# AbrahamSanders/realtime-codec-agent

Hardware: AMD Instinct MI355X
Metric: batch-encode audio-hours/hour (+ xRT and p50 frame-step latency of 1 duplex stream in `duplex`) (higher is better)
Workload: dtype f32; 1 GPU; batch MagiCodec-style encode, 16 kHz stereo, 0.1 s chunks / 2.0 s context, 256 windows per step (BASELINE configs[1]); codebook=131072x16

## Files before the change

realtime_codec_agent_amd/csrc/rca_codec.hip:

```cpp
#include <stdarg.h>

#include <algorithm>
#include <array>
#include <cmath>
#include <map>
#include <type_traits>

#include "rca_common.h"
#include "rca_conv_balance.h"

namespace rca {
thread_local char g_err[512] = {0};
}
using namespace rca;

typedef float f32x16 __attribute__((ext_vector_type(16)));

#define RCA_LAT_MAX_FRAMES 64
#define RCA_LDS_BUDGET (152 * 1024)

typedef float f32x4 __attribute__((ext_vector_type(4)));

struct RowSrc {
    const float* base;
// ... 1864 lines not shown
        float xv[NS][7];
        bool exists[NS];
        int cell[NS];
#pragma unroll
        for (int q = 0; q < NS; ++q) {
            const int tr = tid + 256 * q;
            const int t = t_start + tr;
            exists[q] = tr < WIN && t >= 0 && t < Lin;
            cell[q] = tr < WIN ? (tr % S) * SLOTS + tr / S : -1;
#pragma unroll
            for (int kk = 0; kk < 7; ++kk) {
                const int i = t + kk - 3;
                xv[q][kk] = (tr < WIN && i >= 0 && i < fsrc.T) ? xr[i] : 0.0f;
            }
        }
#pragma unroll
        for (int cb = 0; cb < CPS; ++cb)
#pragma unroll
            for (int h = 0; h < 2; ++h) {
                unsigned hi[NS][4], lo[NS][4];
#pragma unroll
                for (int j = 0; j < 4; ++j) {
                    float v[NS][2];
#pragma unroll
                    for (int e = 0; e < 2; ++e) {
                        const float* wr = w_in8 + (cb * 16 + 8 * h + 2 * j + e) * 8;
                        const float w0 = wr[0], w1 = wr[1], w2 = wr[2], w3 = wr[3], w4 = wr[4], w5 = wr[5], w6 = wr[6], bi = wr[7];
#pragma unroll
                        for (int q = 0; q < NS; ++q) {
                            float a = bi;
#if RCA_BLK_ABL == 1
                            v[q][e] = xv[q][e]; continue;
#endif
                            a = __builtin_fmaf(w0, xv[q][0], a); a = __builtin_fmaf(w1, xv[q][1], a); a = __builtin_fmaf(w2, xv[q][2], a);
                            a = __builtin_fmaf(w3, xv[q][3], a); a = __builtin_fmaf(w4, xv[q][4], a); a = __builtin_fmaf(w5, xv[q][5], a);
                            a = __builtin_fmaf(w6, xv[q][6], a);
                            a = in_act ? fmaxf(a, a * slope) : a;
                            v[q][e] = exists[q] ? a : 0.0f;
                        }
                    }
#pragma unroll
                    for (int q = 0; q < NS; ++q) {
                        hi[q][j] = conv_pack_bf16x2(v[q][0], v[q][1]);
                        if (SPLIT) lo[q][j] = conv_pack_bf16x2(v[q][0] - __uint_as_float(hi[q][j] << 16), v[q][1] - __uint_as_float(hi[q][j] & 0xffff0000u));
                    }
                }
#pragma unroll
                for (int q = 0; q < NS; ++q)
                    if (cell[q] >= 0) {
                        blk_lds[(cb * NPL) * CELLS + h * S * SLOTS + cell[q]] = conv_u32x4{hi[q][0], hi[q][1], hi[q][2], hi[q][3]};
                        if (SPLIT) blk_lds[(cb * NPL + 1) * CELLS + h * S * SLOTS + cell[q]] = conv_u32x4{lo[q][0], lo[q][1], lo[q][2], lo[q][3]};
                    }
            }
    } else {
        stage_load(0);
        stage_write(0);
    }
    __syncthreads();
    int f = 0;
    for (int st = 0; st < nstages; ++st) {
        const int buf = SB ? 0 : (st & 1);
        constexpr int LOAD_AT = CPS * KS - PD;
#pragma unroll
        for (int cb = 0; cb < CPS; ++cb) {
            const conv_u32x4* xb = blk_lds + ((buf * CPS + cb) * NPL) * CELLS;
#pragma unroll
            for (int kk = 0; kk < KS; ++kk) {
                if (cb * KS + kk == LOAD_AT && st + 1 < nstages) stage_load(st + 1);
                const int slot = (cb * KS + kk) % PD;
                const int cell = bcell0 + (kk % S) * SLOTS + kk / S;
                conv_u32x4 bh[4], bl[4];
#pragma unroll
                for (int wn = 0; wn < 4; ++wn) {
                    bh[wn] = xb[cell + wn * 32];
                    if (SPLIT) bl[wn] = xb[CELLS + cell + wn * 32];
                }
                conv_u32x4 a_h[WMT], a_l[WMT];
#pragma unroll
                for (int wm = 0; wm < WMT; ++wm) { a_h[wm] = ah[slot][wm]; if (SPLIT) a_l[wm] = al[slot][wm]; }
                {
                    const long fn = (long)min(f + PD, nfrag - 1) * 64;
#pragma unroll
                    for (int wm = 0; wm < WMT; ++wm) {
                        ah[slot][wm] = wq_hi[wm * wtile + fn];
                        if (SPLIT) al[slot][wm] = wq_lo[wm * wtile + fn];
                    }
                }
                ++f;
#if RCA_BLK_ABL == 2
                asm volatile("" ::"v"(a_h[0]), "v"(bh[0]), "v"(bh[1]), "v"(bh[2]), "v"(bh[3]));
                continue;
#endif
#pragma unroll
                for (int wm = 0; wm < WMT; ++wm)
#pragma unroll
                    for (int wn = 0; wn < 4; ++wn)
                        acc[wm][wn] = __builtin_amdgcn_mfma_f32_32x32x16_bf16(__builtin_bit_cast(conv_bf16x8, a_h[wm]), __builtin_bit_cast(conv_bf16x8, bh[wn]), acc[wm][wn], 0, 0, 0);
                if (SPLIT) {
#pragma unroll
                    for (int wm = 0; wm < WMT; ++wm)
#pragma unroll
                        for (int wn = 0; wn < 4; ++wn)
                            acc[wm][wn] = __builtin_amdgcn_mfma_f32_32x32x16_bf16(__builtin_bit_cast(conv_bf16x8, a_h[wm]), __builtin_bit_cast(conv_bf16x8, bl[wn]), acc[wm][wn], 0, 0, 0);
#pragma unroll
                    for (int wm = 0; wm < WMT; ++wm)
#pragma unroll
                        for (int wn = 0; wn < 4; ++wn)
                            acc[wm][wn] = __builtin_amdgcn_mfma_f32_32x32x16_bf16(__builtin_bit_cast(conv_bf16x8, a_l[wm]), __builtin_bit_cast(conv_bf16x8, bh[wn]), acc[wm][wn], 0, 0, 0);
                }
            }
        }
        if (SB) __syncthreads();
        if (st + 1 < nstages) stage_write(SB ? 0 : (buf ^ 1));
        __syncthreads();
    }
#if RCA_BLK_ABL == 3
    if (lane == 0 && acc[0][0][0] + acc[0][1][1] + acc[WMT - 1][2][2] + acc[WMT - 1][3][3] == 12345.0f) y_hi[0] = 1;
    return;
#endif
#pragma unroll
    for (int wn = 0; wn < 4; ++wn)
#pragma unroll
    for (int wm = 0; wm < WMT; ++wm) {
        const int t = n0 + wn_w * 128 + wn * 32 + n;
        if (t >= Lout) continue;
        if (OUT == 1) {
            float* yr = y_f32 + ((long)b * Cout + co0 + wm * 32 + 4 * half) * Lout + t;
#pragma unroll
            for (int r = 0; r < 16; ++r) yr[(long)((r & 3) + 8 * (r >> 2)) * Lout] = acc[wm][wn][r];
        } else {
            const int Cbo = Cout / 16;
#pragma unroll
            for (int g = 0; g < 4; ++g) {
                float v[4];
#pragma unroll
                for (int j = 0; j < 4; ++j) {
                    const float a = acc[wm][wn][4 * g + j];
                    v[j] = act ? fmaxf(a, a * slope) : a;
                }
                const int ch = co0 + wm * 32 + 8 * g + 4 * half;
                const long o = (((long)b * Cbo + ch / 16) * Lout + t) * 16 + (ch & 15);
                const unsigned h0 = conv_pack_bf16x2(v[0], v[1]), h1 = conv_pack_bf16x2(v[2], v[3]);
                *reinterpret_cast<uint2*>(y_hi + o) = make_uint2(h0, h1);
                if (SPLIT) {
                    const unsigned l0 = conv_pack_bf16x2(v[0] - __uint_as_float(h0 << 16), v[1] - __uint_as_float(h0 & 0xffff0000u));
                    const unsigned l1 = conv_pack_bf16x2(v[2] - __uint_as_float(h1 << 16), v[3] - __uint_as_float(h1 & 0xffff0000u));
                    *reinterpret_cast<uint2*>(y_lo + o) = make_uint2(l0, l1);
                }
            }
        }
    }
}

struct Bf16Pack { conv_bf16raw* hi = nullptr; conv_bf16raw* lo = nullptr; float* w_in8 = nullptr; };

struct rca_codec {
    rca_codec_config_t cfg;
    int device = 0;
    hipStream_t stream = nullptr;
    int hop = 1;
    int variant = 1;
    int mfma_mode = 0;
    bool lat_mode = false;
    int enc_left_frames = 0, dec_left_frames = 0;
    bool window_trim = false;
    std::vector<ConvLayer> enc, dec;
    std::vector<Bf16Pack> bf16_packs;
    bool bf16_blk_split = true;
    float *q_in_w = nullptr, *q_in_b = nullptr;
    float *cb = nullptr, *hc = nullptr, *cbp = nullptr;
    DevBuf act[2], zbuf, keys, io_a, io_b, tail;
    void* pin = nullptr; size_t pin_cap = 0;
    struct StreamGraph { hipGraphExec_t exec = nullptr; int seen = 0; unsigned long long sig = 0; };
    std::map<std::array<int, 5>, StreamGraph> sgraphs;
    bool stream_graphs = true;
    std::map<std::array<long, 4>, float*> ingest_tabs;
    int* err_flag = nullptr;
    hipStream_t last_stream = nullptr;
    bool last_stream_valid = false;
    hipEvent_t xev = nullptr;
    struct Prof { hipEvent_t a, b; int kclass; double flops, bytes; };
    bool profile = false;
    std::vector<Prof> prof;
    std::vector<Prof> prof_pool;
};

struct ProfScope {
    rca_codec* h; hipStream_t st; rca_codec::Prof p; bool on;
    ProfScope(rca_codec* h_, hipStream_t st_, int kclass, double flops, double bytes) : h(h_), st(st_), on(h_->profile) {
        if (!on) return;
        if (!h->prof_pool.empty()) { p = h->prof_pool.back(); h->prof_pool.pop_back(); }
        else { (void)hipEventCreate(&p.a); (void)hipEventCreate(&p.b); }
        p.kclass = kclass; p.flops = flops; p.bytes = bytes;
        (void)hipEventRecord(p.a, st);
    }
    ~ProfScope() {
        if (!on) return;
        (void)hipEventRecord(p.b, st);
        h->prof.push_back(p);
    }
};

static int upload(const rca_tensor_t* ts, int n, const std::string& name, long numel, float** out) {
    const rca_tensor_t* t = find_tensor(ts, n, name);
    if (!t) return fail(RCA_ERR_MISSING, "tensor '%s' missing", name.c_str());
    if (t->numel != numel) return fail(RCA_ERR_ARG, "tensor '%s': numel %ld, expected %ld", name.c_str(), (long)t->numel, numel);
    if (t->dtype != RCA_F32) return fail(RCA_ERR_ARG, "tensor '%s' must be f32", name.c_str());
    RCA_HIP(hipMalloc((void**)out, (size_t)numel * sizeof(float)));
    RCA_HIP(hipMemcpy(*out, t->data, (size_t)numel * sizeof(float), hipMemcpyHostToDevice));
    return RCA_OK;
}

static int pack_weights_cic(const float* w_host, const ConvLayer& L, int cic, float** out, int* nchunks_out) {
    const int K = L.cin * L.k;
    const int nchunks = (L.cin + cic - 1) / cic;
    const int Kpad = nchunks * cic * L.k;
    const int cout_pad = (L.cout + 127) / 128 * 128;
    const long n = (long)(cout_pad / 32) * (Kpad / 8) * 64 * 4;
    std::vector<float> p((size_t)n, 0.0f);
    for (int cot = 0; cot < cout_pad / 32; ++cot)
        for (int q = 0; q < Kpad / 8; ++q)
            for (int lane = 0; lane < 64; ++lane)
                for (int e = 0; e < 4; ++e) {
                    const int co = cot * 32 + (lane & 31);
                    const int k = 2 * (4 * q + e) + (lane >> 5);
                    float v = 0.0f;
                    if (co < L.cout && k < K) v = w_host[(long)co * K + k];
                    p[(((long)cot * (Kpad / 8) + q) * 64 + lane) * 4 + e] = v;
                }
    RCA_HIP(hipMalloc((void**)out, (size_t)n * sizeof(float)));
    RCA_HIP(hipMemcpy(*out, p.data(), (size_t)n * sizeof(float), hipMemcpyHostToDevice));
    *nchunks_out = nchunks;
    return RCA_OK;
}
static int pack_weights(const float* w_host, ConvLayer& L) {
    L.K = L.cin * L.k;
    L.cout_pad = (L.cout + 127) / 128 * 128;
    int rc = pack_weights_cic(w_host, L, conv_cic(L.k, L.s), &L.wp, &L.nchunks);
    if (rc != RCA_OK) return rc;
    L.Kpad = L.nchunks * conv_cic(L.k, L.s) * L.k;
    return pack_weights_cic(w_host, L, conv_cic_ws(L.k, L.s), &L.wp2, &L.nchunks2);
}

static int pack_weights_tr(const float* w_host, ConvLayer& L) {
    const int cic = 16, K = 2 * L.cin;
    const int nchunks = (L.cin + cic - 1) / cic;
    const int Kpad = nchunks * cic * 2;
    L.cout_pad = (L.cout + 127) / 128 * 128;
    const long per_phase = (long)(L.cout_pad / 32) * (Kpad / 8) * 64 * 4;
    std::vector<float> p((size_t)per_phase * L.s, 0.0f);
    for (int r = 0; r < L.s; ++r)
        for (int cot = 0; cot < L.cout_pad / 32; ++cot)
            for (int q = 0; q < Kpad / 8; ++q)
                for (int lane = 0; lane < 64; ++lane)
                    for (int e = 0; e < 4; ++e) {
                        const int co = cot * 32 + (lane & 31);
                        const int k = 2 * (4 * q + e) + (lane >> 5);
                        float v = 0.0f;
                        if (co < L.cout && k < K) {
                            const int ci = k >> 1, j = k & 1;
                            v = w_host[((long)ci * L.cout + co) * L.k + r + j * L.s];
                        }
                        p[r * per_phase + (((long)cot * (Kpad / 8) + q) * 64 + lane) * 4 + e] = v;
                    }
    RCA_HIP(hipMalloc((void**)&L.wp_tr, p.size() * sizeof(float)));
    RCA_HIP(hipMemcpy(L.wp_tr, p.data(), p.size() * sizeof(float), hipMemcpyHostToDevice));
    {
        std::vector<float> t((size_t)L.cin * L.cout * L.k);
        for (int ci = 0; ci < L.cin; ++ci)
            for (int co = 0; co < L.cout; ++co)
                for (int kk = 0; kk < L.k; ++kk) t[((size_t)co * L.k + kk) * L.cin + ci] = w_host[((size_t)ci * L.cout + co) * L.k + kk];
        RCA_HIP(hipMalloc((void**)&L.w_lat, t.size() * sizeof(float)));
        RCA_HIP(hipMemcpy(L.w_lat, t.data(), t.size() * sizeof(float), hipMemcpyHostToDevice));
    }
    L.nchunks_tr = nchunks;
    return RCA_OK;
}

static bool mfma_supported(int k, int s) {
    return (k == 4 && s == 2) || (k == 8 && s == 4) || (k == 10 && s == 5) || (k == 16 && s == 8) || (k == 3 && s == 1);
}

extern "C" const char* rca_last_error(void) { return g_err; }
extern "C" const char* rca_version(void) { return "rca-hip 0.1 (gfx950)"; }
extern "C" int rca_device_sync(int32_t device) {
    RCA_HIP(hipSetDevice(device));
    RCA_HIP(hipDeviceSynchronize());
    return RCA_OK;
}

extern "C" int rca_device_count(int* n) {
    if (!n) return fail(RCA_ERR_ARG, "null");
    RCA_HIP(hipGetDeviceCount(n));
    return RCA_OK;
}

extern "C" int rca_codec_destroy(rca_codec_t* h) {
#ifdef RCA_CONV_TIMELINE
    if (h && getenv("RCA_CONV_TIMELINE_OUT")) {
        long* b = nullptr;
        unsigned n = 6 << 16;
        (void)hipDeviceSynchronize();
        (void)hipMemcpyFromSymbol(&b, HIP_SYMBOL(rca_prof_buf), 8);
        if (b) {
            std::vector<long> host((size_t)(6 << 16) * 8);
            (void)hipMemcpy(host.data(), b, host.size() * 8, hipMemcpyDeviceToHost);
// ... 416 lines not shown
    const double cflops = 2.0 * L.cin * L.k * L.cout * (double)B * Lout;
    const double cbytes = 4.0 * ((double)B * L.cin * Lin + (double)B * L.cout * Lout + (double)L.cin * L.k * L.cout);
    if (view > 0 && view < Lout) {
        const int Lv = view;
        const double vin = std::min((double)Lin, (double)Lv * L.s + L.k - L.s);
        ProfScope ps(h, st, 0, 2.0 * L.cin * L.k * L.cout * (double)B * Lv,
                     4.0 * ((double)B * L.cin * vin + (double)B * L.cout * Lv + (double)L.cin * L.k * L.cout));
        const float* xv = x + (long)(Lout - Lv) * L.s;
        const int act = ((L.pre && !in_activated) ? 1 : 0) | (want_post ? 2 : 0);
        if (post_done) *post_done = want_post;
        if (L.k == 4 && L.s == 2) return launch_conv_mfma<4, 2, 4>(L, xv, y, B, Lin, Lv, slope, st, nullptr, act, 0);
        if (L.k == 8 && L.s == 4) return launch_conv_mfma<8, 4, RCA_CIC_K8>(L, xv, y, B, Lin, Lv, slope, st, nullptr, act, 0);
        if (L.k == 10 && L.s == 5) return launch_conv_mfma<10, 5, 4>(L, xv, y, B, Lin, Lv, slope, st, nullptr, act, 0);
        if (L.k == 16 && L.s == 8) return launch_conv_mfma<16, 8, RCA_CIC_K16>(L, xv, y, B, Lin, Lv, slope, st, nullptr, act, 0);
        if ((long)cdiv((long)B * Lv, 32) * cdiv(L.cout, 32) <= 1024 && L.cin % 16 == 0) {
            launch_conv_cfg<3, 1, 16, 1, 1, 0, 0>(L, L.wp, L.cin / 16, xv, y, Lin, Lv, (long)B * Lv, slope, FuseIn{}, TrInfo{}, st, act);
            RCA_LAUNCH_CHECK();
            return RCA_OK;
        }
        return launch_conv_mfma<3, 1, RCA_CIC_K3>(L, xv, y, B, Lin, Lv, slope, st, nullptr, act, 0);
    }
    if (mfma_conv_ok(h, L, B, Lin, clamp_out)) {
        ProfScope ps(h, st, 0, cflops, cbytes);
        if (h->variant == 2 && try_conv_ws(L, x, y, B, Lin, Lout, slope, st, nullptr)) { RCA_LAUNCH_CHECK(); return RCA_OK; }
        const int act = ((L.pre && !in_activated) ? 1 : 0) | (want_post ? 2 : 0);
        if (post_done) *post_done = want_post;
        if (L.k == 4 && L.s == 2) return launch_conv_mfma<4, 2, 4>(L, x, y, B, Lin, Lout, slope, st, nullptr, act, h->mfma_mode);
        if (L.k == 8 && L.s == 4) return launch_conv_mfma<8, 4, RCA_CIC_K8>(L, x, y, B, Lin, Lout, slope, st, nullptr, act, h->mfma_mode);
        if (L.k == 10 && L.s == 5) return launch_conv_mfma<10, 5, 4>(L, x, y, B, Lin, Lout, slope, st, nullptr, act, h->mfma_mode);
        if (L.k == 16 && L.s == 8) return launch_conv_mfma<16, 8, RCA_CIC_K16>(L, x, y, B, Lin, Lout, slope, st, nullptr, act, h->mfma_mode);
        if (L.k == 3 && L.s == 1) return launch_conv_mfma<3, 1, RCA_CIC_K3>(L, x, y, B, Lin, Lout, slope, st, nullptr, act, h->mfma_mode);
    }
    if (in_activated) return fail(RCA_ERR_ARG, "internal: activated input handed to a kernel without that mode");
    const long total = (long)B * L.cout * Lout;
    ProfScope ps(h, st, 3, cflops, cbytes);
    conv1d_chain_kernel<<<cdiv(total, 256), 256, 0, st>>>(x, L.w, L.b, y, B, L.cin, Lin, L.cout, Lout, L.k, L.s, L.pre, slope, clamp_out);
    RCA_LAUNCH_CHECK();
    return RCA_OK;
}

static int pack_weights_bf16(const ConvLayer& L, Bf16Pack* out) {
    const long nw = (long)L.cout * L.cin * L.k;
    std::vector<float> w(nw);
    RCA_HIP(hipMemcpy(w.data(), L.w, nw * 4, hipMemcpyDeviceToHost));
    const int ncot = L.cout / 32, ncb = L.cin / 16;
    std::vector<conv_bf16raw> hi((size_t)ncot * ncb * L.k * 64 * 8), lo(hi.size());
    auto rne = [](float f) { unsigned u; memcpy(&u, &f, 4); u += 0x7FFFu + ((u >> 16) & 1u); return (conv_bf16raw)(u >> 16); };
    auto up = [](conv_bf16raw h) { unsigned u = (unsigned)h << 16; float f; memcpy(&f, &u, 4); return f; };
    for (int cot = 0; cot < ncot; ++cot)
        for (int cb = 0; cb < ncb; ++cb)
            for (int kk = 0; kk < L.k; ++kk)
                for (int lane = 0; lane < 64; ++lane)
                    for (int j = 0; j < 8; ++j) {
                        const int co = cot * 32 + (lane & 31), ci = cb * 16 + 8 * (lane >> 5) + j;
                        const float v = w[((long)co * L.cin + ci) * L.k + kk];
                        const size_t o = ((((size_t)cot * ncb + cb) * L.k + kk) * 64 + lane) * 8 + j;
                        hi[o] = rne(v);
                        lo[o] = rne(v - up(hi[o]));
                    }
    RCA_HIP(hipMalloc((void**)&out->hi, hi.size() * 2));
    RCA_HIP(hipMalloc((void**)&out->lo, lo.size() * 2));
    RCA_HIP(hipMemcpy(out->hi, hi.data(), hi.size() * 2, hipMemcpyHostToDevice));
    RCA_HIP(hipMemcpy(out->lo, lo.data(), lo.size() * 2, hipMemcpyHostToDevice));
    return RCA_OK;
}

template <int KS, int S, int WGM, int CPS, int OUT, int FUSE = 0, int WMT = 1>
static int launch_conv_bf16(bool split, const ConvLayer& L, const Bf16Pack& wp, const conv_bf16raw* xh, const conv_bf16raw* xl, conv_bf16raw* yh,
                            conv_bf16raw* yl, float* yf, int B, int Lin, int act, float slope, hipStream_t st, RowSrc fsrc = RowSrc{},
                            const float* w_in8 = nullptr, int in_act = 0) {
    constexpr int WGN = 4 / WGM, NT = 128 * WGN;
    constexpr int SLOTS = NT + (KS - 1) / S;
    const int Lout = Lin / S;
    const int n_ct = cdiv(Lout, NT), n_cot = L.cout / (32 * WGM * (split ? 1 : WMT));
    const dim3 grid((unsigned)(((long)n_ct * B + 7) / 8 * 8 * n_cot));
    const int nstages = L.cin / 16 / CPS;
    const size_t lds = (size_t)((nstages > 1 && !(split && S >= 5)) ? 2 : 1) * CPS * (split ? 2 : 1) * 2 * S * SLOTS * 16;
    if (split) {
        auto k = conv_bf16_blk_kernel<KS, S, WGM, CPS, 1, OUT, FUSE, 1>;
        static bool attr = false;
        if (!attr) { (void)hipFuncSetAttribute((const void*)k, hipFuncAttributeMaxDynamicSharedMemorySize, (int)lds); attr = true; }
        k<<<grid, 256, lds, st>>>(xh, xl, wp.hi, wp.lo, L.b, yh, yl, yf, L.cin, Lin, L.cout, Lout, act, slope, B, n_ct, n_cot, fsrc, w_in8, in_act);
    } else {
        auto k = conv_bf16_blk_kernel<KS, S, WGM, CPS, 0, OUT, FUSE, WMT>;
        static bool attr = false;
        if (!attr) { (void)hipFuncSetAttribute((const void*)k, hipFuncAttributeMaxDynamicSharedMemorySize, (int)lds); attr = true; }
        k<<<grid, 256, lds, st>>>(xh, xl, wp.hi, wp.lo, L.b, yh, yl, yf, L.cin, Lin, L.cout, Lout, act, slope, B, n_ct, n_cot, fsrc, w_in8, in_act);
    }
    RCA_LAUNCH_CHECK();
    return RCA_OK;
}

static bool bf16_blk_layer_ok(const ConvLayer& L, bool last) {
    if (L.tr || L.cin % 16 || L.cout % 64) return false;
    if (last) return L.k == 3 && L.s == 1 && L.cin % 64 == 0 && L.cout % 128 == 0;
    if (L.k == 4 && L.s == 2) return L.cin % 32 == 0;
    if ((L.k == 8 && L.s == 4) || (L.k == 10 && L.s == 5) || (L.k == 16 && L.s == 8)) return L.cout % 128 == 0;
    return false;
}
static bool bf16_blk_ok(const rca_codec* h, int tap_layer) {
    const size_t n = h->enc.size();
    if (h->mfma_mode == 0 || h->lat_mode || h->variant != 1 || n < 3) return false;
    if (h->mfma_mode == 3 && !h->bf16_blk_split) return false;
    if (tap_layer >= 0 && tap_layer != (int)n - 1) return false;
    if (h->enc[0].k != 7 || h->enc[0].cin != 1 || h->enc[0].cout % 16 || h->enc[0].cout > 64) return false;
    for (size_t li = 1; li < n; ++li)
        if (!bf16_blk_layer_ok(h->enc[li], li + 1 == n)) return false;
    return true;
}
static int run_encoder_bf16(rca_codec* h, RowSrc src, int B, int Tp, size_t max_elems, hipStream_t st, float** ze_out, int tap_layer, float* tap_dev,
                            int bf16_tap = -1, const conv_bf16raw** bf16_planes = nullptr) {
    const bool split = h->mfma_mode == 3;
    const float slope = h->cfg.leaky_slope;
    const size_t n = h->enc.size();
    int rc;
    if (h->bf16_packs.size() != n) {
        h->bf16_packs.assign(n, Bf16Pack{});
        for (size_t li = 1; li < n; ++li)
            if ((rc = pack_weights_bf16(h->enc[li], &h->bf16_packs[li])) != RCA_OK) return rc;
        const ConvLayer& L0 = h->enc[0];
        std::vector<float> w0((size_t)L0.cout * L0.k), b0(L0.cout), t8((size_t)L0.cout * 8, 0.0f);
        RCA_HIP(hipMemcpy(w0.data(), L0.w, w0.size() * 4, hipMemcpyDeviceToHost));
        RCA_HIP(hipMemcpy(b0.data(), L0.b, b0.size() * 4, hipMemcpyDeviceToHost));
        for (int co = 0; co < L0.cout; ++co) {
            for (int kk = 0; kk < L0.k; ++kk) t8[(size_t)co * 8 + kk] = w0[(size_t)co * L0.k + kk];
            t8[(size_t)co * 8 + 7] = b0[co];
        }
        RCA_HIP(hipMalloc((void**)&h->bf16_packs[0].w_in8, t8.size() * 4));
        RCA_HIP(hipMemcpy(h->bf16_packs[0].w_in8, t8.data(), t8.size() * 4, hipMemcpyHostToDevice));
    }
    auto hi_of = [&](int buf) { return h->act[buf].as<conv_bf16raw>(); };
    auto lo_of = [&](int buf) { return h->act[buf].as<conv_bf16raw>() + max_elems; };
    const double esz = split ? 4.0 : 2.0;
    int cur = 0, L = Tp;
    const bool fuse_in = h->enc[1].k == 4 && h->enc[1].s == 2 && h->enc[0].cout == 32 && !getenv("RCA_BF16_NO_FUSE_IN");
    if (bf16_tap >= 0 && (bf16_tap + 1 >= (int)n || (bf16_tap == 0 && fuse_in)))
        return fail(RCA_ERR_ARG, "bf16 tap: layer %d is not materialised (conv_in fused: %d, last layer: %d, f32)", bf16_tap, (int)fuse_in, (int)n - 1);
    auto stop_at = [&](int li) {
        if (li != bf16_tap) return false;
        bf16_planes[0] = hi_of(cur);
        bf16_planes[1] = lo_of(cur);
        return true;
    };
    if (!fuse_in) {
        const ConvLayer& L0 = h->enc[0];
        const long total = (long)B * L;
        ProfScope ps(h, st, 2, 2.0 * L0.k * L0.cout * (double)total, 4.0 * (double)total + esz * (double)total * L0.cout);
        const int act = h->enc[1].pre ? 1 : 0;
        if (split) conv_in_blk_kernel<7, 1><<<dim3(cdiv(L, 256), B), 256, 0, st>>>(src, h->bf16_packs[0].w_in8, L0.b, hi_of(cur), lo_of(cur), B, L0.cout, L, act, slope);
        else conv_in_blk_kernel<7, 0><<<dim3(cdiv(L, 256), B), 256, 0, st>>>(src, h->bf16_packs[0].w_in8, L0.b, hi_of(cur), lo_of(cur), B, L0.cout, L, act, slope);
        RCA_LAUNCH_CHECK();
        if (stop_at(0)) return RCA_OK;
    }
    for (size_t li = 1; li < n; ++li) {
        const ConvLayer& Ly = h->enc[li];
        const bool last = li + 1 == n;
        const int Lout = L / Ly.s;
        const int act = (!last && h->enc[li + 1].pre) ? 1 : 0;
        const bool fused_li = li == 1 && fuse_in;
        ProfScope ps(h, st, 0, 2.0 * Ly.cin * Ly.k * Ly.cout * (double)B * Lout + (fused_li ? 2.0 * h->enc[0].k * h->enc[0].cout * (double)B * L : 0.0),
                     (fused_li ? 4.0 * (double)B * L : esz * (double)B * Ly.cin * L) + (last ? 4.0 : esz) * (double)B * Ly.cout * Lout +
                         esz * (double)Ly.cin * Ly.k * Ly.cout);
        const Bf16Pack& wp = h->bf16_packs[li];
        const conv_bf16raw *xh = hi_of(cur), *xl = lo_of(cur);
        conv_bf16raw *yh = hi_of(cur ^ 1), *yl = lo_of(cur ^ 1);
        float* yf = h->act[cur ^ 1].as<float>();
        if (!split && Ly.k == 10 && Ly.cout % 256 == 0) rc = launch_conv_bf16<10, 5, 4, 1, 0, 0, 2>(split, Ly, wp, xh, xl, yh, yl, yf, B, L, act, slope, st);
        else if (last) rc = launch_conv_bf16<3, 1, 4, 4, 1>(split, Ly, wp, xh, xl, yh, yl, yf, B, L, act, slope, st);
        else if (Ly.k == 4 && li == 1 && fuse_in)
            rc = launch_conv_bf16<4, 2, 2, 2, 0, 1>(split, Ly, wp, xh, xl, yh, yl, yf, B, L, act, slope, st, src, h->bf16_packs[0].w_in8, Ly.pre ? 1 : 0);
        else if (Ly.k == 4) rc = launch_conv_bf16<4, 2, 2, 2, 0>(split, Ly, wp, xh, xl, yh, yl, yf, B, L, act, slope, st);
        else if (Ly.k == 8) rc = launch_conv_bf16<8, 4, 4, 1, 0>(split, Ly, wp, xh, xl, yh, yl, yf, B, L, act, slope, st);
        else if (Ly.k == 10) rc = launch_conv_bf16<10, 5, 4, 1, 0>(split, Ly, wp, xh, xl, yh, yl, yf, B, L, act, slope, st);
        else rc = launch_conv_bf16<16, 8, 4, 1, 0>(split, Ly, wp, xh, xl, yh, yl, yf, B, L, act, slope, st);
        if (rc != RCA_OK) return rc;
        L = Lout;
        cur ^= 1;
        if (last && tap_layer == (int)li) RCA_HIP(hipMemcpyAsync(tap_dev, yf, (size_t)B * Ly.cout * L * 4, hipMemcpyDeviceToDevice, st));
        if (stop_at((int)li)) return RCA_OK;
    }
    *ze_out = h->act[cur].as<float>();
    return RCA_OK;
}

static int run_encoder(rca_codec* h, RowSrc src, int B, hipStream_t st, float** ze_out, int* F_out, int tap_layer, float* tap_dev,
                       int bf16_tap = -1, const conv_bf16raw** bf16_planes = nullptr, int keep = 0, int* Fz_out = nullptr) {
    const rca_codec_config_t& c = h->cfg;
    const int F = (src.T + h->hop - 1) / h->hop;
    const int Tp = F * h->hop;
    if (F < 1) return fail(RCA_ERR_ARG, "empty audio (T=%d)", src.T);
    if (Fz_out) *Fz_out = F;
    size_t max_elems = 0;
    {
        long L = Tp;
        max_elems = std::max(max_elems, (size_t)B * c.channels[0] * L);
        for (int i = 0; i < c.n_stages; ++i) { L /= c.strides[i]; max_elems = std::max(max_elems, (size_t)B * c.channels[i + 1] * L); }
        max_elems = std::max(max_elems, (size_t)B * c.latent_dim * L);
    }
    int rc;
    if ((rc = h->act[0].ensure(max_elems * 4)) != RCA_OK) return rc;
    if ((rc = h->act[1].ensure(max_elems * 4)) != RCA_OK) return rc;
    if (bf16_blk_ok(h, tap_layer) && (double)B * max_elems < 4.0e18 && Tp / h->enc[1].s >= 64) {
        *F_out = F;
        return run_encoder_bf16(h, src, B, Tp, max_elems, st, ze_out, tap_layer, tap_dev, bf16_tap, bf16_planes);
    }
    if (bf16_tap >= 0) return fail(RCA_ERR_ARG, "bf16 tap: encode() does not take the blocked bf16 pipeline here (mfma mode %d, B=%d T=%d)", h->mfma_mode, B, src.T);
    int cur = 0;
    int L = Tp;
    size_t first = 1;
    const ConvLayer& E0 = h->enc[0];
    const ConvLayer& E1 = h->enc[1];
    const bool fuse01 = !h->lat_mode && h->variant >= 1 && tap_layer != 0 && E0.k == 7 && E1.wp && E1.k == 2 * E1.s && (double)B * E1.cin * L < 4.0e9 &&
                        ((E1.k == 4 && E1.s == 2) || (E1.k == 8 && E1.s == 4) || (E1.k == 16 && E1.s == 8)) && L / E1.s >= 67 &&
                        (double)E1.cout * (L / E1.s) < 2.6e8 &&
                        (src.row_off ? (double)src.span : (double)src.C * (double)std::labs(src.chan_stride) + (double)std::labs(src.win_stride) + src.T) < 5.0e8;
    bool prev_post = false;
    auto handoff = [&](size_t next, int Lnext) {
        return tap_layer < 0 && h->variant == 1 && !h->lat_mode && next < h->enc.size() && h->enc[next].pre && mfma_conv_ok(h, h->enc[next], B, Lnext, 0);
    };
    if (fuse01) {
        float* y = h->act[cur].as<float>();
        FuseIn fin{src, E0.w, E0.b};
        const float slope = c.leaky_slope;
        const int Lout = L / E1.s;
        {
            ProfScope ps(h, st, 0, 2.0 * E1.cin * E1.k * E1.cout * (double)B * Lout + 2.0 * E0.k * E0.cout * (double)B * L,
                         4.0 * ((double)B * src.T + (double)B * E1.cout * Lout + (double)E1.cin * E1.k * E1.cout));
            prev_post = handoff(2, Lout);
            const int act = (E1.pre ? 1 : 0) | (prev_post ? 2 : 0);
            if (h->variant == 2 && try_conv_ws(E1, nullptr, y, B, L, Lout, slope, st, &fin)) { rc = RCA_OK; RCA_LAUNCH_CHECK(); }
            else if (E1.k == 4) rc = launch_conv_mfma<4, 2, 4>(E1, nullptr, y, B, L, Lout, slope, st, &fin, act, h->mfma_mode);
            else if (E1.k == 8) rc = launch_conv_mfma<8, 4, RCA_CIC_K8>(E1, nullptr, y, B, L, Lout, slope, st, &fin, act, h->mfma_mode);
            else rc = launch_conv_mfma<16, 8, RCA_CIC_K16>(E1, nullptr, y, B, L, Lout, slope, st, &fin, act, h->mfma_mode);
        }
        if (rc != RCA_OK) return rc;
        L = Lout;
        first = 2;
        if (tap_layer == 1) RCA_HIP(hipMemcpyAsync(tap_dev, y, (size_t)B * E1.cout * L * 4, hipMemcpyDeviceToDevice, st));
    } else if (h->lat_mode && !src.row_off && src.win_stride == 0 && src.C == B &&
               try_conv_lds(h, h->enc[0], src.base, src.chan_stride, src.T, h->act[cur].as<float>(), B, L, 0, st)) {
        RCA_LAUNCH_CHECK();
    } else {
        const ConvLayer& L0 = h->enc[0];
        const long total = (long)B * L;
        float* y = h->act[cur].as<float>();
        ProfScope ps(h, st, 2, 2.0 * L0.k * L0.cout * (double)total, 4.0 * ((double)total + (double)total * L0.cout));
        if (L0.k == 7) conv_in_kernel<7><<<cdiv(total, 256), 256, 0, st>>>(src, L0.w, L0.b, y, B, L0.cout, L);
        else if (L0.k == 5) conv_in_kernel<5><<<cdiv(total, 256), 256, 0, st>>>(src, L0.w, L0.b, y, B, L0.cout, L);
        else conv_in_kernel<3><<<cdiv(total, 256), 256, 0, st>>>(src, L0.w, L0.b, y, B, L0.cout, L);
        RCA_LAUNCH_CHECK();
        if (tap_layer == 0) RCA_HIP(hipMemcpyAsync(tap_dev, y, (size_t)B * L0.cout * L * 4, hipMemcpyDeviceToDevice, st));
    }
    for (size_t li = first; li < h->enc.size(); ++li) {
        const ConvLayer& Ly = h->enc[li];
        float* x = h->act[cur].as<float>();
        float* y = h->act[cur ^ 1].as<float>();
        bool done = false;
        int view = 0;
        if (li + 1 == h->enc.size() && Fz_out && keep > 0 && tap_layer < 0 && !Ly.tr) {
            const char* hk = getenv("RCA_HEAD_KEEP");
            const int want = keep + conv_view_halo(Ly);
            if (!(hk && hk[0] == '0') && want < L / Ly.s && conv_view_ok(h, Ly, B, L, want)) view = want;
        }
        if ((rc = run_conv(h, Ly, x, y, B, L, 0, st, prev_post, handoff(li + 1, L / Ly.s), &done, view)) != RCA_OK) return rc;
        if (view) *Fz_out = view;
        prev_post = done;
        L /= Ly.s;
        cur ^= 1;
        if (tap_layer == (int)li) RCA_HIP(hipMemcpyAsync(tap_dev, y, (size_t)B * Ly.cout * L * 4, hipMemcpyDeviceToDevice, st));
    }
    *ze_out = h->act[cur].as<float>();
    *F_out = F;
    return RCA_OK;
}

static int run_quantize(rca_codec* h, const float* ze, int ze_is_rows, int B, int F, int f0, int fc, RowDst dst, hipStream_t st,
                        float* ztap_dev) {
    const rca_codec_config_t& c = h->cfg;
    const long rows = (long)B * fc;
    const int J = c.codebook_dim, N = c.codebook_size;
    int rc;
    if ((rc = h->zbuf.ensure((size_t)rows * J * 4)) != RCA_OK) return rc;
    const size_t need_keys = (size_t)rows;
    if (h->keys.cap < need_keys * 8) {
        if ((rc = h->keys.ensure(need_keys * 8)) != RCA_OK) return rc;
        RCA_HIP(hipMemsetAsync(h->keys.p, 0, h->keys.cap, st));
    }
    float* z = h->zbuf.as<float>();
    in_proj_kernel<<<cdiv(rows * J, 256), 256, 0, st>>>(ze, h->q_in_w, h->q_in_b, z, B, c.latent_dim, F, f0, fc, J, ze_is_rows);
    RCA_LAUNCH_CHECK();
    if (ztap_dev) RCA_HIP(hipMemcpyAsync(ztap_dev, z, (size_t)rows * J * 4, hipMemcpyDeviceToDevice, st));
    unsigned long long* keys = h->keys.as<unsigned long long>();
    ProfScope ps(h, st, 1, 2.0 * (double)rows * N * J, 4.0 * ((double)N * (J + 1) + (double)rows * J) + 8.0 * rows);
    if (h->variant >= 1) {
        constexpr int FN = 2;
        const int ftiles = (int)cdiv(rows, FN * 32);
        const int total_tiles = N / 32;
        int splits = (int)std::max(1L, std::min((long)total_tiles / 16, (1024 + ftiles - 1) / (long)ftiles));
        int tps = (total_tiles + splits - 1) / splits;
        tps = (tps + 3) / 4 * 4;
        splits = (total_tiles + tps - 1) / tps;
        dim3 grid(ftiles, splits);
        vq_mfma_kernel<FN><<<grid, 256, 0, st>>>(z, h->cbp, h->hc, keys, rows, N, tps);
    } else {
        constexpr int FB = 4;
        const int fblocks = (int)cdiv(rows, FB);
        int splits = (int)std::max(1L, std::min((long)N / 1024, (1024 + fblocks - 1) / (long)fblocks));
// ... 712 lines not shown
```

Before: 3509 audio-hours/hour.

## Fuse encoder conv_in, k4s2 and k8s4 layers into one bf16 MFMA kernel

Adds a kernel that computes the 7-tap input conv, the first strided k4s2 conv and the second k8s4 conv in one pass. The intermediate activations are kept in LDS as bf16 and never written to global memory. This removes two global round-trips of wide activation tensors and one kernel launch on the non-split bf16 path. In exchange it recomputes halo columns per tile, uses a large LDS footprint that limits occupancy, and can be disabled with an environment variable.

```diff
diff --git a/realtime_codec_agent_amd/csrc/rca_codec.hip b/realtime_codec_agent_amd/csrc/rca_codec.hip
--- a/realtime_codec_agent_amd/csrc/rca_codec.hip
+++ b/realtime_codec_agent_amd/csrc/rca_codec.hip
@@ -2040,6 +2040,188 @@
     }
 }
 
+#define RCA_F12_NT 126
+__global__ __launch_bounds__(256, 2) void conv_bf16_fuse12_kernel(RowSrc fsrc, const float* __restrict__ w_in8, int in_act,
+                                                                  const conv_bf16raw* __restrict__ w1, const float* __restrict__ bias1, int act1,
+                                                                  const conv_bf16raw* __restrict__ w2, const float* __restrict__ bias2, int act2,
+                                                                  conv_bf16raw* __restrict__ y_hi, int L0, int Cout, int Lout, float slope,
+                                                                  int n_rows, int n_ct, int n_cot) {
+    constexpr int NT = RCA_F12_NT, W1 = 4 * NT + 4;
+    static_assert(W1 <= 512 && W1 % 4 == 0 && W1 >= 512 - 4, "four 128-column quarters cover the window; the last one never reads positions 256 / 257");
+    constexpr int SL2 = W1 / 4, HC2 = 4 * SL2;
+    constexpr int MID = 8 * HC2;
+    constexpr int SL1 = 129, HC1 = 2 * SL1;
+    constexpr int PD = 8, NFRAG = 4 * 8;
+    extern __shared__ __attribute__((aligned(16))) conv_u32x4 f12_lds[];
+    conv_u32x4* const mid = f12_lds;
+    conv_u32x4* const xin = f12_lds + MID;
+    const int tid = threadIdx.x, lane = tid & 63, half = lane >> 5, n = lane & 31;
+    const int wave = __builtin_amdgcn_readfirstlane(tid >> 6);
+    const int xcd = blockIdx.x & 7, seq = blockIdx.x >> 3;
+    const int by = seq % n_cot;
+    const int ct = (seq / n_cot) * 8 + xcd;
+    if (ct >= n_ct * n_rows) return;
+    const int b = ct / n_ct;
+    const int n0 = (ct - b * n_ct) * NT;
+    const int co0 = (by * 4 + wave) * 32;
+    const int L1 = L0 / 2;
+    const float s_1 = act1 ? slope : 1.0f, s_2 = act2 ? slope : 1.0f;
+    const int t1s = n0 * 4 - 2;
+    unsigned cv[4][16];
+    {
+        const float* xr = fsrc.base + fsrc.off(b);
+        const int Tm1 = fsrc.T - 1;
+        const int tq = 2 * t1s - 1;
+        float xv[4][7];
+        bool exists[4];
+#pragma unroll
+        for (int q = 0; q < 4; ++q) {
+            const int t0 = tq + 256 * q + tid;
+            exists[q] = t0 >= 0 && t0 < L0;
+#pragma unroll
+            for (int kk = 0; kk < 7; ++kk) {
+                const int i = t0 + kk - 3;
+                const float x = xr[min(max(i, 0), Tm1)];
+                xv[q][kk] = (i >= 0 && i <= Tm1) ? x : 0.0f;
+            }
+        }
+        typedef float f32x2 __attribute__((ext_vector_type(2)));
+        float* const wt = reinterpret_cast<float*>(mid);
+        wt[tid] = w_in8[(2 * (tid >> 4) + (tid & 1)) * 8 + ((tid >> 1) & 7)];
+        __syncthreads();
+        const float s_in = in_act ? slope : 1.0f;
+        const f32x4* wt4 = reinterpret_cast<const f32x4*>(wt);
+        f32x4 pn[4] = {wt4[0], wt4[1], wt4[2], wt4[3]};
+#pragma unroll
+        for (int c2 = 0; c2 < 16; ++c2) {
+            const f32x4 p0 = pn[0], p1 = pn[1], p2 = pn[2], p3 = pn[3];
+            if (c2 < 15) {
+#pragma unroll
+                for (int i = 0; i < 4; ++i) pn[i] = wt4[(c2 + 1) * 4 + i];
+            }
+            asm volatile("" ::: "memory");
+            const f32x2 w0 = {p0[0], p0[1]}, w1_ = {p0[2], p0[3]}, w2_ = {p1[0], p1[1]}, w3 = {p1[2], p1[3]}, w4 = {p2[0], p2[1]}, w5 = {p2[2], p2[3]},
+                        w6 = {p3[0], p3[1]}, bi = {p3[2], p3[3]};
+#pragma unroll
+            for (int q = 0; q < 4; ++q) {
+                f32x2 a = bi;
+                a = __builtin_elementwise_fma(w0, (f32x2){xv[q][0], xv[q][0]}, a);
+                a = __builtin_elementwise_fma(w1_, (f32x2){xv[q][1], xv[q][1]}, a);
+                a = __builtin_elementwise_fma(w2_, (f32x2){xv[q][2], xv[q][2]}, a);
+                a = __builtin_elementwise_fma(w3, (f32x2){xv[q][3], xv[q][3]}, a);
+                a = __builtin_elementwise_fma(w4, (f32x2){xv[q][4], xv[q][4]}, a);
+                a = __builtin_elementwise_fma(w5, (f32x2){xv[q][5], xv[q][5]}, a);
+                a = __builtin_elementwise_fma(w6, (f32x2){xv[q][6], xv[q][6]}, a);
+                const f32x2 m = a * s_in;
+                cv[q][c2] = exists[q] ? conv_pack_bf16x2(fmaxf(a[0], m[0]), fmaxf(a[1], m[1])) : 0u;
+            }
+        }
+    }
+    auto conv_in_write = [&](int q) {
+#pragma unroll
+        for (int cbh = 0; cbh < 4; ++cbh) {
+            xin[cbh * HC1 + (tid & 1) * SL1 + (tid >> 1)] = conv_u32x4{cv[q][4 * cbh], cv[q][4 * cbh + 1], cv[q][4 * cbh + 2], cv[q][4 * cbh + 3]};
+            if (q < 3 && tid < 2) xin[cbh * HC1 + (tid & 1) * SL1 + 128] = conv_u32x4{cv[q + 1][4 * cbh], cv[q + 1][4 * cbh + 1], cv[q + 1][4 * cbh + 2], cv[q + 1][4 * cbh + 3]};
+        }
+    };
+    const conv_u32x4* wq2 = reinterpret_cast<const conv_u32x4*>(w2) + (long)(co0 / 32) * (NFRAG * 64) + lane;
+    conv_u32x4 a2[PD];
+#pragma unroll
+    for (int i = 0; i < PD; ++i) a2[i] = wq2[i * 64];
+    const int wm1 = wave >> 1, wn1 = wave & 1;
+    conv_u32x4 a1[8];
+#pragma unroll
+    for (int i = 0; i < 8; ++i) a1[i] = reinterpret_cast<const conv_u32x4*>(w1)[(wm1 * 8 + i) * 64 + lane];
+    float bv1[16];
+#pragma unroll
+    for (int r = 0; r < 16; ++r) bv1[r] = bias1[wm1 * 32 + (r & 3) + 8 * (r >> 2) + 4 * half];
+    auto k4s2_quarter = [&](int q) {
+        f32x16 acc[2];
+#pragma unroll
+        for (int r = 0; r < 16; ++r) { acc[0][r] = bv1[r]; acc[1][r] = bv1[r]; }
+        const int bcell0 = half * HC1 + wn1 * 64 + n;
+#pragma unroll
+        for (int cb = 0; cb < 2; ++cb)
+#pragma unroll
+            for (int kk = 0; kk < 4; ++kk) {
+                const int cell = cb * 2 * HC1 + bcell0 + (kk % 2) * SL1 + kk / 2;
+                const conv_u32x4 b0 = xin[cell], b1 = xin[cell + 32];
+                acc[0] = __builtin_amdgcn_mfma_f32_32x32x16_bf16(__builtin_bit_cast(conv_bf16x8, a1[cb * 4 + kk]), __builtin_bit_cast(conv_bf16x8, b0), acc[0], 0, 0, 0);
+                acc[1] = __builtin_amdgcn_mfma_f32_32x32x16_bf16(__builtin_bit_cast(conv_bf16x8, a1[cb * 4 + kk]), __builtin_bit_cast(conv_bf16x8, b1), acc[1], 0, 0, 0);
+            }
+#pragma unroll
+        for (int wn = 0; wn < 2; ++wn) {
+            const int c1 = 128 * q + wn1 * 64 + wn * 32 + n;
+            const int t1 = t1s + c1;
+            const bool ok = t1 >= 0 && t1 < L1;
+            if (c1 >= W1) continue;
+            uint2* dst = reinterpret_cast<uint2*>(mid + wm1 * 4 * HC2 + (c1 & 3) * SL2 + (c1 >> 2)) + half;
+#pragma unroll
+            for (int g = 0; g < 4; ++g) {
+                float v[4];
+#pragma unroll
+                for (int j = 0; j < 4; ++j) {
+                    const float a = acc[wn][4 * g + j];
+                    v[j] = fmaxf(a, a * s_1);
+                }
+                const unsigned h0 = conv_pack_bf16x2(v[0], v[1]), h1 = conv_pack_bf16x2(v[2], v[3]);
+                dst[g * HC2 * 2] = ok ? make_uint2(h0, h1) : make_uint2(0u, 0u);
+            }
+        }
+    };
+    conv_in_write(0);
+    __syncthreads();
+#pragma unroll
+    for (int q = 0; q < 4; ++q) {
+        k4s2_quarter(q);
+        __syncthreads();
+        if (q < 3) {
+            conv_in_write(q + 1);
+            __syncthreads();
+        }
+    }
+    f32x16 acc[4];
+#pragma unroll
+    for (int r = 0; r < 16; ++r) {
+        const float bv = bias2[co0 + (r & 3) + 8 * (r >> 2) + 4 * half];
+#pragma unroll
+        for (int wn = 0; wn < 4; ++wn) acc[wn][r] = bv;
+    }
+#pragma unroll
+    for (int cb = 0; cb < 4; ++cb)
+#pragma unroll
+        for (int kk = 0; kk < 8; ++kk) {
+            const int f = cb * 8 + kk;
+            const int cell = (cb * 2 + half) * HC2 + (kk % 4) * SL2 + kk / 4 + n;
+            conv_u32x4 bh[4];
+#pragma unroll
+            for (int wn = 0; wn < 4; ++wn) bh[wn] = mid[cell + wn * 32];
+            const conv_u32x4 a = a2[kk];
+            a2[kk] = wq2[min(f + PD, NFRAG - 1) * 64];
+#pragma unroll
+            for (int wn = 0; wn < 4; ++wn)
+                acc[wn] = __builtin_amdgcn_mfma_f32_32x32x16_bf16(__builtin_bit_cast(conv_bf16x8, a), __builtin_bit_cast(conv_bf16x8, bh[wn]), acc[wn], 0, 0, 0);
+        }
+    const int Cbo = Cout / 16;
+#pragma unroll
+    for (int wn = 0; wn < 4; ++wn) {
+        const int c = wn * 32 + n, t = n0 + c;
+        if (c >= NT || t >= Lout) continue;
+#pragma unroll
+        for (int g = 0; g < 4; ++g) {
+            float v[4];
+#pragma unroll
+            for (int j = 0; j < 4; ++j) {
+                const float a = acc[wn][4 * g + j];
+                v[j] = fmaxf(a, a * s_2);
+            }
+            const int ch = co0 + 8 * g + 4 * half;
+            const long o = (((long)b * Cbo + ch / 16) * Lout + t) * 16 + (ch & 15);
+            *reinterpret_cast<uint2*>(y_hi + o) = make_uint2(conv_pack_bf16x2(v[0], v[1]), conv_pack_bf16x2(v[2], v[3]));
+        }
+    }
+}
+
 struct Bf16Pack { conv_bf16raw* hi = nullptr; conv_bf16raw* lo = nullptr; float* w_in8 = nullptr; };
 
 struct rca_codec {
@@ -2762,7 +2944,32 @@
         RCA_LAUNCH_CHECK();
         if (stop_at(0)) return RCA_OK;
     }
-    for (size_t li = 1; li < n; ++li) {
+    size_t first = 1;
+    {
+        const ConvLayer &E1 = h->enc[1], &E2 = h->enc[2];
+        const char* f12 = getenv("RCA_BF16_FUSE12");
+        const int L2 = L / 2 / 4;
+        if (!split && fuse_in && n > 3 && bf16_tap != 1 && E1.k == 4 && E1.s == 2 && E1.cin == 32 && E1.cout == 64 && E2.k == 8 && E2.s == 4 &&
+            E2.cin == 64 && E2.cout % 128 == 0 && L % 8 == 0 && L2 >= RCA_F12_NT / 2 && !(f12 && f12[0] == '0')) {
+            const ConvLayer& E0 = h->enc[0];
+            ProfScope ps(h, st, 0, 2.0 * E0.k * E0.cout * (double)B * L + 2.0 * E1.cin * E1.k * E1.cout * (double)B * (L / 2) + 2.0 * E2.cin * E2.k * E2.cout * (double)B * L2,
+                         4.0 * (double)B * L + 2.0 * (double)B * E2.cout * L2 + 2.0 * ((double)E1.cin * E1.k * E1.cout + (double)E2.cin * E2.k * E2.cout));
+            const int n_ct = cdiv(L2, RCA_F12_NT), n_cot = E2.cout / 128;
+            const dim3 grid((unsigned)(((long)n_ct * B + 7) / 8 * 8 * n_cot));
+            constexpr size_t lds = (size_t)(8 * (4 * RCA_F12_NT + 4) + 8 * 129) * 16;
+            static bool attr = false;
+            if (!attr) { (void)hipFuncSetAttribute((const void*)conv_bf16_fuse12_kernel, hipFuncAttributeMaxDynamicSharedMemorySize, (int)lds); attr = true; }
+            conv_bf16_fuse12_kernel<<<grid, 256, lds, st>>>(src, h->bf16_packs[0].w_in8, E1.pre ? 1 : 0, h->bf16_packs[1].hi, E1.b, E2.pre ? 1 : 0,
+                                                            h->bf16_packs[2].hi, E2.b, h->enc[3].pre ? 1 : 0, hi_of(cur ^ 1), L, E2.cout, L2, slope,
+                                                            B, n_ct, n_cot);
+            RCA_LAUNCH_CHECK();
+            L = L2;
+            cur ^= 1;
+            first = 3;
+            if (stop_at(2)) return RCA_OK;
+        }
+    }
+    for (size_t li = first; li < n; ++li) {
         const ConvLayer& Ly = h->enc[li];
         const bool last = li + 1 == n;
         const int Lout = L / Ly.s;
```

Result: no change. 3504 audio-hours/hour (-0.1%).
